# berkeley-hipie/HIPIE

Hardware: AMD Instinct MI355X
Metric: images/sec @1024x1024 ViT-H bs=8 (single-image inference hot path: box, class and mask logits) (higher is better)
Workload: dtype f16x3 (split-fp16 operands, fp32 accumulate: fp32-class); 1 GPU; BASELINE.json configs[2]: vit_huge, 1024x1024, batch 8 per GPU, 80 class prompts (L=194), detection; global_batch=8, parallelism=dp1, precision_policy=split, launch=eager

## Files before the change

### hipie_amd/_lib.py

```python
import ctypes
import os

_HERE = os.path.dirname(os.path.abspath(__file__))
LIB_PATH = os.environ.get("HIPIE_LIB_PATH") or os.path.join(_HERE, "csrc", "libhipie_mi355.so")

c_p = ctypes.c_void_p
c_i = ctypes.c_int
c_l = ctypes.c_int64
c_f = ctypes.c_float

SIGNATURES = {
    "hipie_version": [],
    "hipie_last_error": [],
    "hipie_msda_forward": [c_p, c_p, c_p, c_p, c_p, c_p] + [c_i] * 8 + [c_p],
    "hipie_msda_fused_forward": [c_p, c_p, c_p, c_p, c_p, c_p, c_p] + [c_i] * 10 + [c_l, c_l, c_p],
    "hipie_msda_fused_forward_strided": [c_p, c_l, c_p, c_p, c_p, c_p, c_p, c_p] + [c_i] * 10 + [c_l, c_l, c_p],
    "hipie_flash_attn": [c_p, c_p, c_p, c_p] + [c_i] * 5 + [c_l] * 12 + [c_p, c_p, c_i, c_i, c_p, c_f, c_f, c_i, c_p],
    "hipie_vit_attn": [c_p, c_p, c_p, c_p] + [c_i] * 5 + [c_f, c_i, c_p],
    "hipie_vit_attn_fused": [c_p, c_p, c_p, c_p] + [c_i] * 5 + [c_f, c_i, c_p],
    "hipie_vit_attn_rel": [c_p, c_p, c_p, c_p] + [c_i] * 7 + [c_p],
    "hipie_bi_xattn": [c_p, c_p, c_p, c_p, c_p, c_p, c_p] + [c_i] * 5 + [c_f, c_i, c_p],
    "hipie_bi_xattn_ws": [c_p, c_p, c_p, c_p, c_p, c_p, c_p, c_p, c_l] + [c_i] * 5 + [c_f, c_i, c_p],
    "hipie_bi_xattn_workspace": [c_i] * 5,
    "hipie_mask_einsum": [c_p, c_p, c_p] + [c_i] * 6 + [c_p],
    "hipie_mask_einsum_workspace": [c_i, c_i, c_i],
    "hipie_mask_einsum_ws": [c_p, c_p, c_p, c_p, c_p, c_l] + [c_i] * 6 + [c_p],
    "hipie_mask_einsum16": [c_p, c_p, c_p, c_p, c_p] + [c_i] * 6 + [c_p],
    "hipie_dynamic_mask": [c_p, c_p, c_p, c_p] + [c_i] * 7 + [c_p],
    "hipie_dynamic_mask16": [c_p, c_p, c_p, c_p] + [c_i] * 7 + [c_p],
    "hipie_dynamic_mask_backward": [c_p] * 7 + [c_i] * 6 + [c_p],
    "hipie_vit_relpos": [c_p, c_p, c_p, c_p, c_p] + [c_i] * 6 + [c_p],
    "hipie_add_layernorm": [c_p, c_p, c_p, c_p, c_p, c_p, c_l, c_i, c_f, c_i, c_i, c_i, c_p],
    "hipie_add_layernorm_sum": [c_p, c_p, c_p, c_p, c_p, c_p, c_p, c_p, c_l, c_i, c_f, c_i, c_i, c_i, c_p],
    "hipie_add_layernorm_rows": [c_p, c_p, c_p, c_p, c_p, c_p, c_l, c_i, c_f, c_i, c_i, c_i, c_p, c_p, c_p],
    "hipie_batched_nms": [c_p, c_p, c_p, c_p, c_p, c_i, c_i, c_f, c_i, c_p],
    "hipie_mask_finalize": [c_p, c_i, c_p] + [c_i] * 8 + [c_f, c_p, c_p],
    "hipie_sem_pan": [c_p] * 8 + [c_i] * 11 + [c_p],
    "hipie_sine_embed": [c_p, c_p, c_p, c_l, c_i, c_i, c_i, c_f, c_i, c_p],
    "hipie_box_refine": [c_p, c_p, c_p, c_l, c_f, c_i, c_p],
    "hipie_ref_point_mlp": [c_p, c_p, c_p, c_p, c_p, c_p, c_p, c_l, c_i, c_f, c_i, c_p],
    "hipie_box_head": [c_p, c_p, c_p, c_p, c_p, c_p, c_p, c_p, c_p, c_l, c_f, c_p],
    "hipie_add_layernorm_dec": [c_p, c_p, c_p, c_p, c_p, c_p, c_p, c_p, c_l, c_i, c_f, c_i, c_i, c_p],
    "hipie_add_cast": [c_p, c_p, c_p, c_l, c_i, c_p],
    "hipie_group_norm": [c_p, c_p, c_p, c_p, c_p, c_p, c_i, c_i, c_i, c_i, c_i, c_f, c_i, c_i, c_i, c_p],
    "hipie_gemm": [c_p, c_l, c_p, c_l, c_p, c_p, c_l, c_p, c_l, c_p] + [c_i] * 6 + [c_f, c_f, c_p],
    "hipie_gemm_f8x": [c_p, c_l, c_p, c_l, c_p, c_p, c_p, c_l, c_p, c_l, c_p] + [c_i] * 6 + [c_f, c_f, c_p],
    "hipie_to_f8x": [c_p, c_l, c_p, c_l, c_p, c_l, c_i, c_p],
    "hipie_gemm_ln": [c_p, c_l, c_p, c_l, c_p, c_p, c_l, c_p, c_p, c_f, c_p, c_l, c_p, c_l, c_i, c_i, c_i, c_f, c_p],
    "hipie_gemm_gather": [c_p, c_l, c_l, c_p, c_p, c_l, c_p, c_p, c_l, c_p, c_l, c_p] + [c_i] * 6 + [c_f, c_f, c_p],
    "hipie_vit_attn_split": [c_p, c_p, c_p, c_p] + [c_i] * 5 + [c_p],
    "hipie_msda_backward": [c_p] * 9 + [c_i] * 8 + [c_p],
    "hipie_msda_backward_ws": [c_p] * 9 + [c_i] * 8 + [c_p, c_l, c_p],
    "hipie_msda_backward_workspace": [c_i] * 6,
    "hipie_gemm_batched": [c_p, c_l, c_l, c_l, c_p, c_l, c_l, c_l, c_p, c_l, c_l, c_l] + [c_i] * 6 + [c_f, c_p],
    "hipie_gemm_batched_softmax_bias": [c_p, c_l, c_l, c_l, c_p, c_l, c_l, c_l, c_p, c_l, c_l, c_l] + [c_i] * 5 + [c_p, c_i, c_p, c_f, c_f, c_p],
    "hipie_gemm_batched_resid": [c_p, c_l, c_l, c_l, c_p, c_l, c_l, c_l, c_p, c_p, c_l, c_l, c_l, c_p, c_l, c_l, c_l] + [c_i] * 5 + [c_f, c_p],
    "hipie_gemm_batched_softmax": [c_p, c_l, c_l, c_l, c_p, c_l, c_l, c_l, c_p, c_l, c_l, c_l] + [c_i] * 5 + [c_p, c_i, c_f, c_f, c_p],
    "hipie_softmax_hl8": [c_p, c_l, c_p, c_l, c_l, c_i, c_i, c_p, c_l, c_f, c_p],
    "hipie_attn_f32": [c_p] * 5 + [c_i] * 5 + [c_l] * 6 + [c_f, c_p],
    "hipie_attn_split": [c_p] * 5 + [c_i] * 5 + [c_l] * 6 + [c_f, c_p],
    "hipie_attn_f32_rows": [c_p] * 5 + [c_i] * 5 + [c_l] * 6 + [c_f, c_p],
    "hipie_attn_split_rows": [c_p] * 5 + [c_i] * 5 + [c_l] * 6 + [c_f, c_p],
    "hipie_conv3x3_split": [c_p, c_l, c_p, c_p, c_p, c_l, c_l] + [c_i] * 6 + [c_p],
    "hipie_ffn_fused": [c_p, c_l, c_p, c_p, c_p, c_p, c_p, c_l, c_i, c_i, c_i, c_p],
    "hipie_topk": [c_p, c_l, c_i, c_i, c_i, c_p, c_p, c_p],
    "hipie_fill_rows": [c_p, c_l, c_p, c_l, c_p, c_l, c_p],
    "hipie_to_hl8": [c_p, c_l, c_p, c_l, c_l, c_i, c_i, c_f, c_p],
    "hipie_to_hl8_t": [c_p, c_l, c_p, c_l, c_l, c_i, c_l, c_f, c_p],
    "hipie_attn_train_forward": [c_p] * 8 + [c_i, c_i, c_p],
    "hipie_to_f16_pair": [c_p, c_l, c_p, c_p, c_l, c_i, c_i, c_p, c_p],
    "hipie_attn_train_backward": [c_p] * 13 + [c_i, c_i, c_p],
    "hipie_selftest": [c_i, c_p, c_p, c_p, c_p],
}

_lib = None


class HipieLibraryError(RuntimeError):
    pass


def load():
    global _lib
    if _lib is not None:
        return _lib
    if not os.path.exists(LIB_PATH):
        raise HipieLibraryError(
            "libhipie_mi355.so not found at %s -- build it with `make -C hipie_amd/csrc` (hipcc, gfx950). "
            "There is no PyTorch fallback for the hand-written kernels." % LIB_PATH)
    import torch
    try:
        lib = ctypes.CDLL(LIB_PATH)
    except OSError as e:
        raise HipieLibraryError("cannot load %s: %s" % (LIB_PATH, e))
    for name, argtypes in SIGNATURES.items():
        try:
            fn = getattr(lib, name)
        except AttributeError:
            raise HipieLibraryError("%s does not export %s (stale build?)" % (LIB_PATH, name))
        fn.argtypes = argtypes
        fn.restype = (ctypes.c_char_p if name == "hipie_last_error" else
                      ctypes.c_int64 if name in ("hipie_bi_xattn_workspace", "hipie_mask_einsum_workspace", "hipie_msda_backward_workspace") else ctypes.c_int)
    _lib = lib
    return lib


def check(rc, what):
    if rc != 0:
        msg = load().hipie_last_error()
        raise RuntimeError("%s failed (rc=%d): %s" % (what, rc, msg.decode() if msg else ""))
```

### hipie_amd/csrc/ffn_fused.hip

```cpp
#include "common.h"
#include "mfma.h"

namespace hipie {

struct FFParams {
  const char* X; const char* W1; const char* W2; const float* b1; const float* b2; float* out;
  long ldx_b, ldw1_b, ldw2_b, ldo;
  int M;
};

__device__ __forceinline__ void ff_dma16(const char* sbase, unsigned int voff, unsigned int lds_dst) {
#if defined(__HIP_DEVICE_COMPILE__)
  unsigned int keep;
  asm volatile("s_mov_b32 %0, m0\n\ts_mov_b32 m0, %3\n\ts_nop 0\n\tglobal_load_lds_dwordx4 %1, %2\n\ts_mov_b32 m0, %0"
               : "=&s"(keep) : "v"(voff), "s"(sbase), "s"(lds_dst) : "memory");
#endif
}

constexpr int FF_D = 256, FF_F = 2048, FF_C = 32;
constexpr int FF_W1B = FF_C * FF_D * 4;
constexpr int FF_W2B = FF_D * FF_C * 4;
constexpr int FF_BUF = FF_W1B + FF_W2B;

__global__ __launch_bounds__(256, 1) void ffn_fused_kernel(const FFParams p) {
  typedef f16_t T;
  typedef Mfma32<T>::frag frag;
  constexpr int KS = FF_D / 16;
  constexpr int NB = FF_D / 32;
  constexpr int NCH = FF_F / FF_C;
  extern __shared__ __attribute__((aligned(1024))) char smem[];
  float* sb1 = reinterpret_cast<float*>(smem + 2 * FF_BUF);

  const int tid = threadIdx.x, lane = tid & 63;
  const int wave = __builtin_amdgcn_readfirstlane(tid >> 6);
  const int li = lane & 31, hi = lane >> 5;
  const int m = blockIdx.x * 128 + wave * 32 + li;
  const int mc = min(m, p.M - 1);

  for (int i = tid; i < FF_F / 4; i += 256) reinterpret_cast<float4*>(sb1)[i] = reinterpret_cast<const float4*>(p.b1)[i];

  frag xh[KS], xl[KS];
  {
    const char* xr = p.X + (long)mc * p.ldx_b + 32 * hi;
#pragma unroll
    for (int ks = 0; ks < KS; ++ks) {
      xh[ks] = *reinterpret_cast<const frag*>(xr + 64 * ks);
      xl[ks] = *reinterpret_cast<const frag*>(xr + 64 * ks + 16);
    }
  }

  unsigned int dv1[8], dv2[8];
#pragma unroll
  for (int q = 0; q < 8; ++q) {
    const int i = wave + 4 * q;
    dv1[q] = (unsigned int)((long)i * p.ldw1_b + 16 * (lane ^ (i & 15)));
    const int f = 8 * i + (lane >> 3);
    dv2[q] = (unsigned int)((long)f * p.ldw2_b + 16 * ((lane & 7) ^ ((f >> 1) & 7)));
  }
  const unsigned int lds0 = (unsigned int)reinterpret_cast<uintptr_t>((__attribute__((address_space(3))) char*)smem);
  auto dma_chunk = [&](const int c, const int buf, const int q) {
    const int i = wave + 4 * q;
    ff_dma16(p.W1 + (long)c * FF_C * p.ldw1_b, dv1[q], __builtin_amdgcn_readfirstlane(lds0 + (unsigned int)(buf * FF_BUF + 1024 * i)));
    ff_dma16(p.W2 + (long)c * (FF_C * 4), dv2[q], __builtin_amdgcn_readfirstlane(lds0 + (unsigned int)(buf * FF_BUF + FF_W1B + 1024 * i)));
  };

  f32x16 acc[NB];
#pragma unroll
  for (int j = 0; j < NB; ++j)
#pragma unroll
    for (int r = 0; r < 16; ++r) acc[j][r] = 0.f;

#pragma unroll
  for (int q = 0; q < 8; ++q) dma_chunk(0, 0, q);

  const int w1row = li * 1024, w1sw = li & 15;
  const int w2row = FF_W1B + li * 128, w2sw = (li >> 1) & 7;

  for (int c = 0; c < NCH; ++c) {
    const int buf = c & 1;
    __builtin_amdgcn_s_waitcnt(0x0F70);
    __syncthreads();
    const char* bs = smem + buf * FF_BUF;
    const bool more = c + 1 < NCH;

    f32x16 h0, h1;
#pragma unroll
    for (int r = 0; r < 16; ++r) { h0[r] = 0.f; h1[r] = 0.f; }
#pragma unroll
    for (int ks = 0; ks < KS; ks += 2) {
      const frag ah0 = *reinterpret_cast<const frag*>(bs + w1row + 16 * ((2 * (2 * ks + hi)) ^ w1sw));
      const frag al0 = *reinterpret_cast<const frag*>(bs + w1row + 16 * ((2 * (2 * ks + hi) + 1) ^ w1sw));
      const frag ah1 = *reinterpret_cast<const frag*>(bs + w1row + 16 * ((2 * (2 * ks + 2 + hi)) ^ w1sw));
      const frag al1 = *reinterpret_cast<const frag*>(bs + w1row + 16 * ((2 * (2 * ks + 2 + hi) + 1) ^ w1sw));
      h0 = Mfma32<T>::mma(al0, xh[ks], h0);
      h1 = Mfma32<T>::mma(al1, xh[ks + 1], h1);
      h0 = Mfma32<T>::mma(ah0, xl[ks], h0);
      h1 = Mfma32<T>::mma(ah1, xl[ks + 1], h1);
      h0 = Mfma32<T>::mma(ah0, xh[ks], h0);
      h1 = Mfma32<T>::mma(ah1, xh[ks + 1], h1);
      if (more) dma_chunk(c + 1, buf ^ 1, ks >> 1);
    }
    frag Hh[2], Hl[2];
#pragma unroll
    for (int g = 0; g < 4; ++g) {
      const float4 b4 = *reinterpret_cast<const float4*>(sb1 + c * FF_C + 8 * g + 4 * hi);
      const float bb[4] = {b4.x, b4.y, b4.z, b4.w};
#pragma unroll
      for (int e = 0; e < 4; ++e) {
        const int r = 4 * g + e;
        T hh, ll;
        hl_split(fmaxf(h0[r] + h1[r] + bb[e], 0.f), hh, ll);
        Hh[r >> 3][r & 7] = hh;
        Hl[r >> 3][r & 7] = ll;
      }
    }
#pragma unroll
    for (int s2 = 0; s2 < 2; ++s2) {
      frag wh[NB], wl[NB];
#pragma unroll
      for (int j = 0; j < NB; ++j) {
        wh[j] = *reinterpret_cast<const frag*>(bs + w2row + j * 4096 + 16 * ((2 * (2 * s2 + hi)) ^ w2sw));
        wl[j] = *reinterpret_cast<const frag*>(bs + w2row + j * 4096 + 16 * ((2 * (2 * s2 + hi) + 1) ^ w2sw));
      }
#pragma unroll
      for (int j = 0; j < NB; ++j) acc[j] = Mfma32<T>::mma(wl[j], Hh[s2], acc[j]);
#pragma unroll
      for (int j = 0; j < NB; ++j) acc[j] = Mfma32<T>::mma(wh[j], Hl[s2], acc[j]);
#pragma unroll
      for (int j = 0; j < NB; ++j) acc[j] = Mfma32<T>::mma(wh[j], Hh[s2], acc[j]);
    }
  }

  if (m < p.M) {
    float* orow = p.out + (long)m * p.ldo;
#pragma unroll
    for (int j = 0; j < NB; ++j)
#pragma unroll
      for (int g = 0; g < 4; ++g) {
        const int n = 32 * j + 8 * g + 4 * hi;
        const float4 b4 = *reinterpret_cast<const float4*>(p.b2 + n);
        *reinterpret_cast<float4*>(orow + n) = make_float4(acc[j][4 * g] + b4.x, acc[j][4 * g + 1] + b4.y, acc[j][4 * g + 2] + b4.z, acc[j][4 * g + 3] + b4.w);
      }
  }
}

}

extern "C" int hipie_ffn_fused(const void* x, int64_t ldx, const void* w1, const float* b1, const void* w2p, const float* b2, float* out,
                               int64_t ldo, int M, int D, int F, void* stream) {
  using namespace hipie;
  HIPIE_REQUIRE(x && w1 && b1 && w2p && b2 && out, "ffn_fused: null pointer");
  HIPIE_REQUIRE(D == FF_D && F == FF_F, "ffn_fused: model width %d / hidden width %d (built for 256 / 2048)", D, F);
  HIPIE_REQUIRE(M > 0 && ldx >= 2 * D && ldx % 8 == 0 && ldo >= D && ldo % 4 == 0, "ffn_fused: M=%d ldx=%ld ldo=%ld", M, (long)ldx, (long)ldo);
  HIPIE_REQUIRE((((uintptr_t)x | (uintptr_t)w1 | (uintptr_t)w2p | (uintptr_t)b1 | (uintptr_t)b2 | (uintptr_t)out) & 15) == 0,
                "ffn_fused: pointers must be 16-byte aligned");
  FFParams p;
  p.X = (const char*)x; p.W1 = (const char*)w1; p.W2 = (const char*)w2p; p.b1 = b1; p.b2 = b2; p.out = out;
  p.ldx_b = ldx * 2; p.ldw1_b = (long)2 * D * 2; p.ldw2_b = (long)2 * F * 2; p.ldo = ldo;
  p.M = M;
  const size_t lds = (size_t)2 * FF_BUF + FF_F * sizeof(float);
  static bool lds_set[64] = {false};
  int dev = 0;
  (void)hipGetDevice(&dev);
  if (dev < 0 || dev >= 64 || !lds_set[dev]) {
    (void)hipFuncSetAttribute((const void*)ffn_fused_kernel, hipFuncAttributeMaxDynamicSharedMemorySize, (int)lds);
    if (dev >= 0 && dev < 64) lds_set[dev] = true;
  }
  hipLaunchKernelGGL(ffn_fused_kernel, dim3((unsigned)((M + 127) / 128)), dim3(256), lds, (hipStream_t)stream, p);
  return check_launch("ffn_fused");
}
```

### hipie_amd/ops.py

```python
import torch

from . import _lib

_DT = {torch.float32: 0, torch.float16: 1, torch.bfloat16: 2}
F32, F16, BF16, HL8 = 0, 1, 2, 4
OUT_F32 = 0x100
K_HL8_HI = 0x200


class _Profile(object):

    def __init__(self):
        self.tags, self.events = set(), {}
        self.shapes = False

    def enable(self, *tags):
        self.tags, self.events = set(tags), {}

    def disable(self):
        self.tags = set()

    def begin(self, tag):
        if tag not in self.tags and "all" not in self.tags:
            return None
# ... 1009 lines not shown
        lead = (M,)
        if out is not None and out_row is None and out.numel() // out.shape[-1] < M:
            raise RuntimeError("gemm: `out` has fewer rows (%d) than the row map (%d)" % (out.numel() // out.shape[-1], M))
        if resid is not None and resid.numel() // N < M:
            raise RuntimeError("gemm: `resid` has fewer rows (%d) than the row map (%d)" % (resid.numel() // N, M))
    if out_row is not None:
        if out is None:
            lead = (int(out_rows),)
        if out_row.dtype != torch.int32 or out_row.numel() != M or not out_row.is_contiguous():
            raise RuntimeError("gemm: out_row must be a contiguous int32 vector with one entry per row of a")
    if out is None:
        if out_fmt == F32:
            out = torch.empty(*lead, N, dtype=torch.float32, device=a.device)
        elif out_fmt == F16:
            out = torch.empty(*lead, N, dtype=torch.float16, device=a.device)
        else:
            out = torch.empty(*lead, 2 * N, dtype=torch.float16, device=a.device)
    o2 = out.reshape(-1, out.shape[-1])
    r2 = None
    if resid is not None:
        r2 = resid.reshape(-1, N)
        if r2.dtype != torch.float32 or r2.stride(-1) != 1:
            raise RuntimeError("gemm: resid must be fp32 with contiguous rows")
    if bias is not None and (bias.dtype != torch.float32 or not bias.is_contiguous()):
        raise RuntimeError("gemm: bias must be contiguous fp32")
    if a_row is not None:
        rc = lib.hipie_gemm_gather(a2.data_ptr(), a2.stride(0), a2.shape[0], a_row.data_ptr(), _chk(w, "w"), w.shape[1],
                                   None if bias is None else bias.data_ptr(), None if r2 is None else r2.data_ptr(), 0 if r2 is None else r2.stride(0),
                                   o2.data_ptr(), o2.stride(0), None if out_row is None else out_row.data_ptr(), M, N, Kw,
                                   F32 if a_f32 else HL8, int(out_fmt), int(act), float(alpha), float(oscale), _stream())
        _lib.check(rc, "hipie_gemm_gather")
        return out
    rc = lib.hipie_gemm(a2.data_ptr(), a2.stride(0), _chk(w, "w"), w.shape[1], None if bias is None else bias.data_ptr(),
                        None if r2 is None else r2.data_ptr(), 0 if r2 is None else r2.stride(0), o2.data_ptr(), o2.stride(0),
                        None if out_row is None else out_row.data_ptr(), M, N, Kw, F32 if a_f32 else (HL8 if split else F16), int(out_fmt), int(act), float(alpha), float(oscale), _stream())
    _lib.check(rc, "hipie_gemm")
    return out


@_timed(lambda qkv, tab_h, tab_w, grid_hw, heads: "vit_attn_global" if grid_hw[0] * grid_hw[1] > 256 else "vit_attn_window")
def vit_attn_split(qkv, tab_h, tab_w, grid_hw, heads):
    lib = _lib.load()
    gh, gw = grid_hw
    B, N, C6 = qkv.shape
    hd = C6 // (6 * heads)
    if qkv.dtype != torch.float16 or tab_h.dtype != torch.float16 or tab_w.dtype != torch.float16:
        raise RuntimeError("vit_attn_split: HL8 (fp16) operands expected")
    out = torch.empty(B, N, 2 * heads * hd, dtype=torch.float16, device=qkv.device)
    rc = lib.hipie_vit_attn_split(_chk(qkv, "qkv"), _chk(tab_h, "tab_h"), _chk(tab_w, "tab_w"), out.data_ptr(), B, gh, gw, heads, hd, _stream())
    _lib.check(rc, "hipie_vit_attn_split")
    return out


@_timed("gemm_split_k")
def gemm_split_k(a_hl8, w_hl8, nk):
    lib = _lib.load()
    M, K2 = a_hl8.shape
    N = w_hl8.shape[0]
    K = K2 // 2
    if w_hl8.shape[1] != K2 or K % (32 * nk) or a_hl8.dtype != torch.float16 or w_hl8.dtype != torch.float16 or not a_hl8.is_cuda:
        raise RuntimeError("gemm_split_k: HL8 device operands (M, 2K) / (N, 2K), K a multiple of 32 * nk")
    if N % 8:
        raise RuntimeError("gemm_split_k: N must be a multiple of 8")
    Kc = K // nk
    part = torch.empty(nk, M, N, dtype=torch.float32, device=a_hl8.device)
    rc = lib.hipie_gemm_batched(a_hl8.data_ptr(), K2, 0, 2 * Kc, w_hl8.data_ptr(), K2, 0, 2 * Kc, part.data_ptr(), N, 0, M * N, 1, nk, M, N, Kc,
                                F32, 1.0, _stream())
    _lib.check(rc, "hipie_gemm_batched")
    return part.sum(0)


@_timed("gemm_batched")
def matmul_nt_batched(a, w, alpha=1.0):
    lib = _lib.load()
    B, M, K = a.shape
    N = w.shape[1]
    if w.shape[0] != B or w.shape[2] != K or K % 32 or not a.is_cuda:
        raise RuntimeError("matmul_nt_batched: a (B, M, K), w (B, N, K) device tensors with K %% 32 == 0, got %s / %s" % (tuple(a.shape), tuple(w.shape)))
    Np = (N + 7) // 8 * 8
    if Np != N:
        wp = torch.zeros(B, Np, K, dtype=torch.float32, device=w.device)
        wp[:, :N] = w
        w = wp
    ah, wh = to_hl8(a.float().contiguous()), to_hl8(w.float().contiguous())
    out = torch.empty(B, M, Np, dtype=torch.float32, device=a.device)
    rc = lib.hipie_gemm_batched(ah.data_ptr(), 2 * K, M * 2 * K, 0, wh.data_ptr(), 2 * K, Np * 2 * K, 0, out.data_ptr(), Np, M * Np, 0,
                                B, 1, M, Np, K, F32, float(alpha), _stream())
    _lib.check(rc, "hipie_gemm_batched")
    return out if Np == N else out[..., :N]


def vit_attn_split_ok(grid_hw, hd):
    gh, gw = grid_hw

    def rows_ok(kh, kw):
        return (kw <= 32 and kh <= 160) or (kw <= 64 and kh <= 132) or (64 < kw <= 96 and kh <= 160)
    return hd in (64, 80) and ((gw == 14 and gh <= 96) or rows_ok(gh, gw) or (gw > 96 and gh <= 96 and rows_ok(gw, gh)))


def split_weight(owner, key, params, weight_fn, bias_fn=None):
    ver = tuple((q.data_ptr(), q._version, str(q.device)) for q in params)
    cache = owner.__dict__.setdefault("_hl8_cache", {})
    e = cache.get(key)
    if e is None or e[0] != ver:
        w = weight_fn().detach().float()
        b = None if bias_fn is None else bias_fn()
        b = None if b is None else b.detach().float()
        N = w.shape[0]
        Np = (N + 7) // 8 * 8
        if Np != N:
            w = torch.nn.functional.pad(w, (0, 0, 0, Np - N))
            b = None if b is None else torch.nn.functional.pad(b, (0, Np - N))
        e = (ver, hl8_pack(w), None if b is None else b.contiguous(), N)
        cache[key] = e
    return e[1], e[2], e[3]


def conv3x3_split_ok(x, conv):
    return (x.is_cuda and x.dim() == 4 and conv.kernel_size == (3, 3) and conv.stride == (1, 1) and conv.padding == (1, 1) and conv.dilation == (1, 1)
            and conv.padding_mode == "zeros" and conv.groups == 1 and conv.weight.dtype == torch.float32 and conv.in_channels % 32 == 0 and conv.out_channels % 256 == 0
            and x.shape[0] * (x.shape[2] + 2) * (x.shape[3] + 2) >= 16384)


_CONV_STAGE = {}
_RETIRED = []


@_timed("conv3x3_split")
def conv3x3_split(x, conv, act=ACT_NONE):
    lib = _lib.load()
    B, C, H, W = x.shape
    N = conv.out_channels
    Hp, Wp = H + 2, W + 2
    guard = Wp + 1
    rows = B * Hp * Wp
    skey = (B, C, H, W, str(x.device), torch.cuda.current_stream(x.device).cuda_stream)
    buf = _CONV_STAGE.get(skey)
    if buf is None:
        if len(_CONV_STAGE) >= 8:
            _RETIRED.append(_CONV_STAGE.pop(next(iter(_CONV_STAGE))))
        buf = _CONV_STAGE[skey] = torch.zeros(rows + 2 * guard, C, dtype=torch.float32, device=x.device)
    buf[guard:guard + rows].view(B, Hp, Wp, C)[:, 1:-1, 1:-1].copy_(x.permute(0, 2, 3, 1))
    w, b, _ = split_weight(conv, "w3x3", [conv.weight] + ([conv.bias] if conv.bias is not None else []),
                           lambda: conv.weight.permute(0, 2, 3, 1).reshape(N, 9 * C), (lambda: conv.bias) if conv.bias is not None else None)
    out = torch.empty(rows, N, dtype=torch.float32, device=x.device)
    xin = buf[guard:]
    rc = lib.hipie_conv3x3_split(xin.data_ptr(), C, w.data_ptr(), None if b is None else b.data_ptr(), out.data_ptr(), N, rows, Wp, C, N,
                                 F32, F32, int(act), _stream())
    _lib.check(rc, "hipie_conv3x3_split")
    return out.view(B, Hp, Wp, N)[:, 1:-1, 1:-1].permute(0, 3, 1, 2).contiguous(memory_format=torch.channels_last)


_FFN_PERM = {}


def ffn_fused_ok(x_hl8, lin1, lin2):
    return (x_hl8.is_cuda and lin1.weight.shape == (2048, 256) and lin2.weight.shape == (256, 2048) and lin1.bias is not None
            and lin2.bias is not None and lin1.weight.dtype == torch.float32 and x_hl8.numel() // 512 >= 4096)


@_timed("ffn_fused")
def ffn_fused(x_hl8, lin1, lin2):
    lib = _lib.load()
    w1, b1, _ = split_weight(lin1, "w", [lin1.weight, lin1.bias], lambda: lin1.weight, lambda: lin1.bias)
    F_ = lin2.weight.shape[1]
    perm = _FFN_PERM.get(F_)
    if perm is None:
        base = torch.tensor([0, 1, 2, 3, 8, 9, 10, 11, 4, 5, 6, 7, 12, 13, 14, 15])
        perm = _FFN_PERM[F_] = (torch.arange(0, F_, 16)[:, None] + base[None, :]).reshape(-1)
    w2, b2, _ = split_weight(lin2, "w_ffn_perm", [lin2.weight, lin2.bias], lambda: lin2.weight[:, perm.to(lin2.weight.device)], lambda: lin2.bias)
    lead = x_hl8.shape[:-1]
    x2 = x_hl8.reshape(-1, x_hl8.shape[-1])
    if x2.dtype != torch.float16 or x2.stride(-1) != 1 or x2.shape[-1] != 512:
        raise RuntimeError("ffn_fused: x must be HL8 rows of 2 * 256 fp16 values")
    M = x2.shape[0]
    out = torch.empty(M, 256, dtype=torch.float32, device=x2.device)
    rc = lib.hipie_ffn_fused(x2.data_ptr(), x2.stride(0), w1.data_ptr(), b1.data_ptr(), w2.data_ptr(), b2.data_ptr(), out.data_ptr(), 256,
                             M, 256, F_, _stream())
    _lib.check(rc, "hipie_ffn_fused")
    return out.view(*lead, 256)


def split_ok(K):
    return K % 32 == 0


def split_linear(x, owner, key, weight, bias=None, act=ACT_NONE, out_fmt=F32, resid=None, x_hl8=False, weight_fn=None, bias_fn=None,
                 tag="gemm", params=None, out=None, out_row=None, a_row=None):
    if params is None:
        params = [weight] + ([bias] if bias is not None else [])
    w, b, N = split_weight(owner, key, params, weight_fn or (lambda: weight), bias_fn or ((lambda: bias) if bias is not None else None))
    if x_hl8:
        a = x
    elif x.dtype == torch.float32 and x.stride(-1) == 1 and x.data_ptr() % 16 == 0 and (x.dim() < 2 or x.stride(-2) % 4 == 0):
        a = x if x.dim() <= 2 or x.is_contiguous() else x.contiguous()
    else:
        a = to_hl8(x if x.dtype in (torch.float32, torch.float16) else x.float())
    if out is not None or out_row is not None or a_row is not None:
        if N != w.shape[0]:
            raise RuntimeError("split_linear: in-place / row-mapped outputs need N % 8 == 0")
        return gemm(a, w, b, resid, out_fmt=out_fmt, act=act, split=True, tag=tag, out=out, out_row=out_row, a_row=a_row)
    out = gemm(a, w, b, resid, out_fmt=out_fmt, act=act, split=True, tag=tag)
    if N != w.shape[0]:
        out = out[..., :(2 * N if out_fmt == HL8 else N)].contiguous()
    return out



@_timed("to_f8x")
def to_f8x(x_hl8):
    lib = _lib.load()
    if x_hl8.dtype != torch.float16 or not x_hl8.is_cuda or x_hl8.shape[-1] % 64:
        raise RuntimeError("to_f8x: HL8 rows (fp16, 2K columns with K a multiple of 32) on the device")
    x2 = x_hl8.reshape(-1, x_hl8.shape[-1])
    if x2.stride(-1) != 1:
        x2 = x2.contiguous()
    R, K = x2.shape[0], x2.shape[1] // 2
    q = torch.empty(R, 2 * K, dtype=torch.uint8, device=x_hl8.device)
    sc = torch.empty(R, K // 32, 2, dtype=torch.uint8, device=x_hl8.device)
    rc = lib.hipie_to_f8x(x2.data_ptr(), x2.stride(0), q.data_ptr(), 2 * K, sc.data_ptr(), R, K, _stream())
    _lib.check(rc, "hipie_to_f8x")
    return q, sc


def f8x_weight(owner, key, params, weight_fn, bias_fn=None):
    from . import fp8x
    ver = tuple((q.data_ptr(), q._version, str(q.device)) for q in params)
    cache = owner.__dict__.setdefault("_f8x_cache", {})
    e = cache.get(key)
    if e is None or e[0] != ver:
        w = weight_fn().detach().float()
        b = None if bias_fn is None else bias_fn()
        b = None if b is None else b.detach().float()
        N = w.shape[0]
        Np = (N + 7) // 8 * 8
        if Np != N:
            w = torch.nn.functional.pad(w, (0, 0, 0, Np - N))
            b = None if b is None else torch.nn.functional.pad(b, (0, Np - N))
        w_hl8 = hl8_pack(w)
        q, sc = to_f8x(w_hl8) if w_hl8.is_cuda else (None, None)
        w8, wsc = fp8x.pack_from_hl8(w_hl8, q, sc)
        e = (ver, w8, wsc, None if b is None else b.contiguous(), N)
        cache[key] = e
    return e[1], e[2], e[3], e[4]


@_timed("gemm_f8x")
def gemm_f8x(a, w8, wsc, bias=None, resid=None, out_fmt=F32, act=ACT_NONE, alpha=1.0, oscale=1.0, out=None, out_row=None, out_rows=None):
    lib = _lib.load()
    if a.dtype != torch.float16 or w8.dtype != torch.uint8 or wsc.dtype != torch.uint8 or not a.is_cuda:
        raise RuntimeError("gemm_f8x: a HL8 (fp16) rows, w8 / wsc uint8, on the device")
    N, K = w8.shape[0], w8.shape[1] // 4
    a2 = a if a.dim() == 2 else a.reshape(-1, a.shape[-1])
    if a2.stride(-1) != 1 or a2.shape[-1] != 2 * K or not w8.is_contiguous() or tuple(wsc.shape) != (N, K // 32, 2) or not wsc.is_contiguous():
        raise RuntimeError("gemm_f8x: a rows %s against an f8x weight %s / scales %s" % (tuple(a.shape), tuple(w8.shape), tuple(wsc.shape)))
    M = a2.shape[0]
    lead = a.shape[:-1]
    if out_row is not None:
        if out is None:
            lead = (int(out_rows),)
        if out_row.dtype != torch.int32 or out_row.numel() != M or not out_row.is_contiguous():
            raise RuntimeError("gemm_f8x: out_row must be a contiguous int32 vector with one entry per row of a")
    if out is None:
        dt, width = {F32: (torch.float32, N), F16: (torch.float16, N), HL8: (torch.float16, 2 * N)}[out_fmt]
        out = torch.empty(*lead, width, dtype=dt, device=a.device)
    o2 = out.reshape(-1, out.shape[-1])
    r2 = None
    if resid is not None:
        r2 = resid.reshape(-1, N)
        if r2.dtype != torch.float32 or r2.stride(-1) != 1:
            raise RuntimeError("gemm_f8x: resid must be fp32 with contiguous rows")
    if bias is not None and (bias.dtype != torch.float32 or not bias.is_contiguous()):
        raise RuntimeError("gemm_f8x: bias must be contiguous fp32")
    rc = lib.hipie_gemm_f8x(a2.data_ptr(), a2.stride(0), _chk(w8, "w8"), 2 * K, _chk(wsc, "wsc"), None if bias is None else bias.data_ptr(),
                            None if r2 is None else r2.data_ptr(), 0 if r2 is None else r2.stride(0), o2.data_ptr(), o2.stride(0),
                            None if out_row is None else out_row.data_ptr(), M, N, K, HL8, int(out_fmt), int(act), float(alpha), float(oscale), _stream())
    _lib.check(rc, "hipie_gemm_f8x")
    return out


def f8x_linear(x_hl8, owner, key, weight, bias=None, act=ACT_NONE, out_fmt=F32, resid=None, out=None):
    params = [weight] + ([bias] if bias is not None else [])
    w8, wsc, b, N = f8x_weight(owner, key, params, lambda: weight, (lambda: bias) if bias is not None else None)
    if N != w8.shape[0]:
        raise RuntimeError("f8x_linear: N %% 8 == 0 expected (got %d)" % N)
    return gemm_f8x(x_hl8, w8, wsc, b, resid, out_fmt=out_fmt, act=act, out=out)

def split_linear_ln_ok(x, weight, norm_weight):
    return (x.is_cuda and weight.dtype == torch.float32 and weight.shape[0] == 256 and norm_weight.numel() == 256 and weight.shape[1] % 32 == 0
            and not torch.is_grad_enabled())


@_timed("gemm_ln")
def split_linear_ln(x, owner, key, weight, bias, resid, norm_weight, norm_bias, eps, x_hl8=False, want_hl8=True):
    lib = _lib.load()
    w, b, N = split_weight(owner, key, [weight] + ([bias] if bias is not None else []), lambda: weight, (lambda: bias) if bias is not None else None)
    if N != 256 or w.shape[0] != 256:
        raise RuntimeError("split_linear_ln: 256 output features expected")
    K = w.shape[1] // 2
    a_f32 = not x_hl8
    if a_f32 and (x.dtype != torch.float32 or x.stride(-1) != 1):
        raise RuntimeError("split_linear_ln: x must be fp32 rows or HL8")
    a2 = x.reshape(-1, x.shape[-1])
    if a2.shape[-1] != (K if a_f32 else 2 * K) or (a_f32 and (a2.stride(0) % 4 or a2.data_ptr() % 16)):
        raise RuntimeError("split_linear_ln: operand rows %s against weight %s" % (tuple(x.shape), tuple(weight.shape)))
    r2 = resid.reshape(-1, 256)
    M = a2.shape[0]
    if r2.dtype != torch.float32 or r2.stride(-1) != 1 or r2.shape[0] != M or not r2.is_cuda:
        raise RuntimeError("split_linear_ln: resid must be (rows, 256) fp32 on the device")
    out = torch.empty(*resid.shape[:-1], 256, dtype=torch.float32, device=x.device)
    o16 = torch.empty(*resid.shape[:-1], 512, dtype=torch.float16, device=x.device) if want_hl8 else None
    rc = lib.hipie_gemm_ln(a2.data_ptr(), a2.stride(0), _chk(w, "w"), w.shape[1], None if b is None else b.data_ptr(), r2.data_ptr(), r2.stride(0),
                           _chk(norm_weight, "norm_weight", torch.float32), _chk(norm_bias, "norm_bias", torch.float32), float(eps),
                           out.data_ptr(), 256, None if o16 is None else o16.data_ptr(), 512, M, K, F32 if a_f32 else HL8, 1.0, _stream())
    _lib.check(rc, "hipie_gemm_ln")
    return out, o16


_SHUFFLE_MAPS = {}


def _shuffle_maps(B, H, W, device):
    key = (B, H, W, str(device))
    m = _SHUFFLE_MAPS.get(key)
    if m is None:
        b = torch.arange(B, device=device).view(B, 1, 1)
        h = torch.arange(H, device=device).view(1, H, 1)
        w = torch.arange(W, device=device).view(1, 1, W)
        m = [((b * 2 * H + 2 * h + i) * 2 * W + 2 * w + j).reshape(-1).to(torch.int32).contiguous() for i in range(2) for j in range(2)]
        if len(_SHUFFLE_MAPS) > 16:
            _RETIRED.extend(_SHUFFLE_MAPS.values())
# ... 36 lines not shown
```

### include/hipie_mi355.h

```cpp
#ifndef HIPIE_MI355_H
#define HIPIE_MI355_H

#include <stdint.h>

#ifdef __cplusplus
extern "C" {
#endif

#define HIPIE_ABI_VERSION 13

#define HIPIE_F32 0
#define HIPIE_F16 1
#define HIPIE_BF16 2
#define HIPIE_F64 3
#define HIPIE_HL8 4

#define HIPIE_OUT_F32 0x100
#define HIPIE_K_HL8_HI 0x200

#define HIPIE_ATTN_FAST 1

#define HIPIE_OK 0
#define HIPIE_EINVAL (-22)
#define HIPIE_ELAUNCH (-5)
// ... 34 lines not shown

int hipie_vit_attn(const void* qkv, const float* rel_h, const float* rel_w, void* out,
                   int B, int gh, int gw, int heads, int hd, float scale, int dtype, void* stream);

int hipie_bi_xattn(const void* q, const void* k, const void* vv, const void* vl, const uint8_t* text_mask,
                   void* out_v, void* out_l, int B, int H, int Nv, int L, int hd, float clamp, int dtype, void* stream);

int64_t hipie_bi_xattn_workspace(int B, int H, int Nv, int L, int head_dim);
int hipie_bi_xattn_ws(const void* q, const void* k, const void* vv, const void* vl, const uint8_t* text_mask,
                      void* out_v, void* out_l, void* workspace, int64_t workspace_bytes, int B, int H, int Nv, int L,
                      int head_dim, float clamp, int dtype, void* stream);

int hipie_mask_einsum(const float* embed, const float* feats, void* out, int B, int Q, int C, int HW,
                      int precision, int out_dtype, void* stream);

int64_t hipie_mask_einsum_workspace(int B, int Q, int C);
int hipie_mask_einsum_ws(const float* embed, const float* feats, const float* row_bias, void* out, void* workspace,
                         int64_t workspace_bytes, int B, int Q, int C, int HW, int precision, int out_dtype, void* stream);

int hipie_mask_einsum16(const void* embed_hi, const void* embed_lo, const void* feats, const float* row_bias, void* out, int B,
                        int Q, int C, int HW, int dtype, int out_dtype, void* stream);

int hipie_dynamic_mask(const float* feats, const float* refs, const float* params, void* out,
                       int B, int Q, int H, int W, int stride, int up, int out_dtype, void* stream);

int hipie_dynamic_mask_backward(const float* feats, const float* refs, const float* params, const float* grad_out, float* grad_feats,
                                float* grad_refs, float* grad_params, int B, int Q, int H, int W, int stride, int up, void* stream);

int hipie_dynamic_mask16(const float* feats, const float* refs, const float* params, void* out,
                         int B, int Q, int H, int W, int stride, int dtype, int out_dtype, void* stream);

int hipie_vit_relpos(const void* qkv, const void* tab_h, const void* tab_w, float* rel_h, float* rel_w,
                     int B, int gh, int gw, int heads, int hd, int dtype, void* stream);

int hipie_add_layernorm(const void* x, const void* delta, const float* gamma, const float* beta, void* res_out,
                        void* norm_out, int64_t rows, int C, float eps, int x_dtype, int delta_dtype, int norm_dtype,
                        void* stream);

int hipie_vit_attn_fused(const void* qkv, const void* tab_h, const void* tab_w, void* out, int B, int gh, int gw, int heads,
                         int hd, float scale, int dtype, void* stream);

int hipie_vit_attn_rel(const void* qkv, const void* tab_h, const void* tab_w, void* out, int B, int gh, int gw, int heads,
                       int hd, int dtype, int flags, void* stream);

int hipie_add_layernorm_rows(const void* x, const void* delta, const float* gamma, const float* beta, void* res_out,
                             void* norm_out, int64_t out_rows, int C, float eps, int x_dtype, int delta_dtype,
                             int norm_dtype, const int32_t* delta_row, const int32_t* out_src, void* stream);

int hipie_add_layernorm_sum(const void* x, const void* delta, const float* gamma, const float* beta, void* res_out,
                            void* norm_out, const void* addend, void* sum_out, int64_t rows, int C, float eps,
                            int x_dtype, int delta_dtype, int norm_dtype, void* stream);

int hipie_add_layernorm_dec(const float* x, const void* delta, const float* gamma, const float* beta, float* norm_out,
                            void* norm16_out, const void* addend, void* sum16_out, int64_t rows, int C, float eps,
                            int delta_dtype, int aux_dtype, void* stream);

int hipie_ref_point_mlp(const float* ref, const float* dim_t, const void* w1t, const void* b1, const void* w2t, const void* b2,
                        void* out, int64_t n, int ref_stride, float scale, int dtype, void* stream);
int hipie_box_head(const float* x, const float* ref, const float* w1t, const float* b1, const float* w2t, const float* b2,
                   const float* w3t, const float* b3, float* out, int64_t n, float eps, void* stream);

int hipie_group_norm(const void* x, const float* prebias, const float* gamma, const float* beta, void* out, float* workspace,
                     int B, int C, int HW, int groups, int channels_last, float eps, int relu, int x_dtype, int out_dtype,
                     void* stream);

int hipie_add_cast(const float* a, const void* b, void* out, int64_t n, int dtype, void* stream);

int hipie_batched_nms(const float* boxes, const int64_t* classes, const int32_t* order, int32_t* keep, int32_t* count,
                      int B, int Q, float iou_threshold, int coordinate_trick, void* stream);

int hipie_mask_finalize(const void* masks, int dtype, const int32_t* qidx, int n, int hm, int wm, int up, int crop_h,
                        int crop_w, int out_h, int out_w, float threshold, uint8_t* out, void* stream);

int hipie_sem_pan(const float* masks, const void* cls_hi, const void* cls_lo, const float* pscore, float* sem,
                  int32_t* pan_idx, uint8_t* pan_own, int32_t* area, int N, int Npad, int C, int hm, int wm, int up,
                  int crop_h, int crop_w, int out_h, int out_w, int precision, void* stream);

int hipie_sine_embed(const float* ref, const float* dim_t, void* out, int64_t n, int n_coord, int num_pos_feats, int ref_stride,
                     float scale, int out_dtype, void* stream);

int hipie_box_refine(const void* delta, const float* ref, float* out, int64_t n, float eps, int delta_dtype, void* stream);

int hipie_gemm(const void* A, int64_t lda, const void* W, int64_t ldw, const float* bias, const float* resid, int64_t ldr,
               void* out, int64_t ldo, const int32_t* out_row, int M, int N, int K, int in_fmt, int out_fmt, int act, float alpha,
               float oscale, void* stream);

int hipie_gemm_f8x(const void* A, int64_t lda, const void* W, int64_t ldw, const void* w_scale, const float* bias, const float* resid,
                   int64_t ldr, void* out, int64_t ldo, const int32_t* out_row, int M, int N, int K, int in_fmt, int out_fmt, int act,
                   float alpha, float oscale, void* stream);

int hipie_to_f8x(const void* x, int64_t ldx, void* out, int64_t ldo, void* scale, int64_t rows, int K, void* stream);

int hipie_gemm_ln(const void* A, int64_t lda, const void* W, int64_t ldw, const float* bias, const float* resid, int64_t ldr,
                  const float* gamma, const float* beta, float eps, float* out, int64_t ldo, void* out_hl8, int64_t ldo_hl8, int M, int K,
                  int in_fmt, float alpha, void* stream);

int hipie_gemm_gather(const void* A, int64_t lda, int64_t a_rows, const int32_t* a_row, const void* W, int64_t ldw, const float* bias,
                      const float* resid, int64_t ldr, void* out, int64_t ldo, const int32_t* out_row, int M, int N, int K, int in_fmt,
                      int out_fmt, int act, float alpha, float oscale, void* stream);

int hipie_vit_attn_split(const void* qkv, const void* tab_h, const void* tab_w, void* out, int B, int gh, int gw, int heads,
                         int hd, void* stream);

int hipie_attn_train_forward(const void* q_hi, const void* q_lo, const void* k_hi, const void* k_lo, const void* v_hi, const void* v_lo,
                             void* out, void* lse, int BH, int N, void* stream);
int hipie_to_f16_pair(const void* x, int64_t ldx, void* hi, void* lo, int64_t rows, int C, int Cp, const void* scale, void* stream);
int hipie_attn_train_backward(const void* q_hi, const void* q_lo, const void* k_hi, const void* k_lo, const void* v_hi, const void* v_lo,
                              const void* do_hi, const void* do_lo, const void* lse, const void* delta, void* dq, void* dk, void* dv,
                              int BH, int N, void* stream);

int hipie_fill_rows(void* dst, int64_t ld_bytes, const int32_t* rows, int64_t n_rows, const void* src_row, int64_t row_bytes, void* stream);

int hipie_to_hl8(const void* x, int64_t ldx, void* out, int64_t ldo, int64_t rows, int K, int x_dtype, float scale, void* stream);

int hipie_to_hl8_t(const void* x, int64_t ldx, void* out, int64_t ldo, int64_t rows, int C, int64_t rows_p, float scale, void* stream);

int hipie_gemm_batched(const void* A, int64_t lda, int64_t a_outer, int64_t a_inner, const void* W, int64_t ldw, int64_t w_outer,
                       int64_t w_inner, void* out, int64_t ldo, int64_t o_outer, int64_t o_inner, int n_outer, int n_inner, int M, int N,
                       int K, int out_fmt, float alpha, void* stream);

int hipie_gemm_batched_softmax(const void* A, int64_t lda, int64_t a_outer, int64_t a_inner, const void* W, int64_t ldw, int64_t w_outer,
                               int64_t w_inner, void* out, int64_t ldo, int64_t o_outer, int64_t o_inner, int n_outer, int n_inner, int M,
                               int N, int K, const unsigned char* mask, int L, float clamp, float alpha, void* stream);

int hipie_gemm_batched_softmax_bias(const void* A, int64_t lda, int64_t a_outer, int64_t a_inner, const void* W, int64_t ldw, int64_t w_outer,
                                    int64_t w_inner, void* out, int64_t ldo, int64_t o_outer, int64_t o_inner, int n_outer, int n_inner,
                                    int M, int N, int K, const unsigned char* mask, int L, const float* col_bias, float clamp, float alpha,
                                    void* stream);
int hipie_gemm_batched_resid(const void* A, int64_t lda, int64_t a_outer, int64_t a_inner, const void* W, int64_t ldw, int64_t w_outer,
                             int64_t w_inner, const float* bias, const float* resid, int64_t ldr, int64_t r_outer, int64_t r_inner, float* out,
                             int64_t ldo, int64_t o_outer, int64_t o_inner, int n_outer, int n_inner, int M, int N, int K, float alpha,
                             void* stream);

int hipie_softmax_hl8(const float* S, int64_t lds, void* P, int64_t ldp, int64_t rows, int L, int Lp, const unsigned char* mask,
                      int64_t rows_per_batch, float clamp, void* stream);

int hipie_attn_f32(const float* q, const float* k, const float* v, const unsigned char* key_mask, float* out, int B, int H, int Nq, int Nk,
                   int head_dim, int64_t q_sb, int64_t q_st, int64_t k_sb, int64_t k_st, int64_t v_sb, int64_t v_st, float scale,
                   void* stream);

int hipie_attn_f32_rows(const float* q, const float* k, const float* v, const unsigned char* query_mask, float* out, int B, int H, int Nq,
                        int Nk, int head_dim, int64_t q_sb, int64_t q_st, int64_t k_sb, int64_t k_st, int64_t v_sb, int64_t v_st, float scale,
                        void* stream);
int hipie_attn_split_rows(const float* q, const float* k, const float* v, const unsigned char* query_mask, float* out, int B, int H, int Nq,
                          int Nk, int head_dim, int64_t q_sb, int64_t q_st, int64_t k_sb, int64_t k_st, int64_t v_sb, int64_t v_st, float scale,
                          void* stream);

int hipie_attn_split(const float* q, const float* k, const float* v, const unsigned char* key_mask, float* out, int B, int H, int Nq, int Nk,
                   int head_dim, int64_t q_sb, int64_t q_st, int64_t k_sb, int64_t k_st, int64_t v_sb, int64_t v_st, float scale,
                   void* stream);

int hipie_ffn_fused(const void* x, int64_t ldx, const void* w1, const float* b1, const void* w2p, const float* b2, float* out, int64_t ldo,
                    int M, int D, int F, void* stream);

int hipie_conv3x3_split(const void* x, int64_t ldx, const void* w, const float* bias, void* out, int64_t ldo, int64_t rows, int Wp, int C,
                        int N, int in_fmt, int out_fmt, int act, void* stream);

int hipie_topk(const float* x, int64_t row_stride, int rows, int n, int k, int64_t* idx_out, float* val_out, void* stream);

int hipie_selftest(int which, const uint16_t* a, const uint16_t* b, float* out, void* stream);

#ifdef __cplusplus
}
#endif
#endif
```

Baseline: 41.91 images/sec.

## Split tail tiles of fused FFN across hidden chunks with atomic reduction

```diff
diff --git a/hipie_amd/_lib.py b/hipie_amd/_lib.py
--- a/hipie_amd/_lib.py
+++ b/hipie_amd/_lib.py
@@ -63,6 +63,8 @@
     "hipie_attn_split_rows": [c_p] * 5 + [c_i] * 5 + [c_l] * 6 + [c_f, c_p],
     "hipie_conv3x3_split": [c_p, c_l, c_p, c_p, c_p, c_l, c_l] + [c_i] * 6 + [c_p],
     "hipie_ffn_fused": [c_p, c_l, c_p, c_p, c_p, c_p, c_p, c_l, c_i, c_i, c_i, c_p],
+    "hipie_ffn_fused_workspace": [c_i],
+    "hipie_ffn_fused_ws": [c_p, c_l, c_p, c_p, c_p, c_p, c_p, c_l, c_i, c_i, c_i, c_p, c_l, c_p],
     "hipie_topk": [c_p, c_l, c_i, c_i, c_i, c_p, c_p, c_p],
     "hipie_fill_rows": [c_p, c_l, c_p, c_l, c_p, c_l, c_p],
     "hipie_to_hl8": [c_p, c_l, c_p, c_l, c_l, c_i, c_i, c_f, c_p],
@@ -100,7 +102,8 @@
             raise HipieLibraryError("%s does not export %s (stale build?)" % (LIB_PATH, name))
         fn.argtypes = argtypes
         fn.restype = (ctypes.c_char_p if name == "hipie_last_error" else
-                      ctypes.c_int64 if name in ("hipie_bi_xattn_workspace", "hipie_mask_einsum_workspace", "hipie_msda_backward_workspace") else ctypes.c_int)
+                      ctypes.c_int64 if name in ("hipie_bi_xattn_workspace", "hipie_mask_einsum_workspace", "hipie_msda_backward_workspace",
+                                                  "hipie_ffn_fused_workspace") else ctypes.c_int)
     _lib = lib
     return lib
 
diff --git a/hipie_amd/csrc/ffn_fused.hip b/hipie_amd/csrc/ffn_fused.hip
--- a/hipie_amd/csrc/ffn_fused.hip
+++ b/hipie_amd/csrc/ffn_fused.hip
@@ -7,6 +7,8 @@
   const char* X; const char* W1; const char* W2; const float* b1; const float* b2; float* out;
   long ldx_b, ldw1_b, ldw2_b, ldo;
   int M;
+  int nfull, S;
+  float* part; unsigned int* cnt;
 };
 
 __device__ __forceinline__ void ff_dma16(const char* sbase, unsigned int voff, unsigned int lds_dst) {
@@ -34,7 +36,12 @@
   const int tid = threadIdx.x, lane = tid & 63;
   const int wave = __builtin_amdgcn_readfirstlane(tid >> 6);
   const int li = lane & 31, hi = lane >> 5;
-  const int m = blockIdx.x * 128 + wave * 32 + li;
+  const int bid = blockIdx.x;
+  const int tt = bid < p.nfull ? -1 : (bid - p.nfull) / p.S;
+  const int piece = bid < p.nfull ? 0 : (bid - p.nfull) - tt * p.S;
+  const int tile = bid < p.nfull ? bid : p.nfull + tt;
+  const int c0 = tt < 0 ? 0 : piece * NCH / p.S, c1 = tt < 0 ? NCH : (piece + 1) * NCH / p.S;
+  const int m = tile * 128 + wave * 32 + li;
   const int mc = min(m, p.M - 1);
 
   for (int i = tid; i < FF_F / 4; i += 256) reinterpret_cast<float4*>(sb1)[i] = reinterpret_cast<const float4*>(p.b1)[i];
@@ -71,17 +78,16 @@
     for (int r = 0; r < 16; ++r) acc[j][r] = 0.f;
 
 #pragma unroll
-  for (int q = 0; q < 8; ++q) dma_chunk(0, 0, q);
+  for (int q = 0; q < 8; ++q) dma_chunk(c0, 0, q);
 
   const int w1row = li * 1024, w1sw = li & 15;
   const int w2row = FF_W1B + li * 128, w2sw = (li >> 1) & 7;
 
-  for (int c = 0; c < NCH; ++c) {
-    const int buf = c & 1;
+  auto chunk = [&](const int c, const bool more) __attribute__((always_inline)) {
+    const int buf = (c - c0) & 1;
     __builtin_amdgcn_s_waitcnt(0x0F70);
     __syncthreads();
     const char* bs = smem + buf * FF_BUF;
-    const bool more = c + 1 < NCH;
 
     f32x16 h0, h1;
 #pragma unroll
@@ -129,6 +135,54 @@
 #pragma unroll
       for (int j = 0; j < NB; ++j) acc[j] = Mfma32<T>::mma(wh[j], Hh[s2], acc[j]);
     }
+  };
+  for (int c = c0; c < c1 - 1; ++c) chunk(c, true);
+  chunk(c1 - 1, false);
+
+  if (tt >= 0) {
+    auto partial = [&](const int s) { return reinterpret_cast<float4*>(p.part) + (long)(tt * p.S + s) * (NB * 4 * 256) + tid; };
+    float4* mine = partial(piece);
+#pragma unroll
+    for (int j = 0; j < NB; ++j)
+#pragma unroll
+      for (int g = 0; g < 4; ++g) mine[(4 * j + g) * 256] = make_float4(acc[j][4 * g], acc[j][4 * g + 1], acc[j][4 * g + 2], acc[j][4 * g + 3]);
+    asm volatile("s_waitcnt vmcnt(0)" ::: "memory");
+    __syncthreads();
+    int* flag = reinterpret_cast<int*>(sb1);
+    if (tid == 0) {
+      __builtin_amdgcn_fence(__ATOMIC_RELEASE, "agent");
+      asm volatile("s_waitcnt vmcnt(0)" ::: "memory");
+      const bool last = __hip_atomic_fetch_add(p.cnt + tt, 1u, __ATOMIC_RELAXED, __HIP_MEMORY_SCOPE_AGENT) == (unsigned int)(p.S - 1);
+      if (last) {
+        __builtin_amdgcn_fence(__ATOMIC_ACQUIRE, "agent");
+        asm volatile("s_waitcnt vmcnt(0)" ::: "memory");
+      }
+      *flag = last;
+    }
+    __syncthreads();
+    if (!*flag) return;
+    if (m >= p.M) return;
+    float4 t[NB * 4];
+#pragma unroll
+    for (int i = 0; i < NB * 4; ++i) t[i] = partial(0)[i * 256];
+    for (int s = 1; s < p.S; ++s) {
+      float4 f[NB * 4];
+#pragma unroll
+      for (int i = 0; i < NB * 4; ++i) f[i] = partial(s)[i * 256];
+#pragma unroll
+      for (int i = 0; i < NB * 4; ++i) { t[i].x += f[i].x; t[i].y += f[i].y; t[i].z += f[i].z; t[i].w += f[i].w; }
+    }
+    float* orow = p.out + (long)m * p.ldo;
+#pragma unroll
+    for (int j = 0; j < NB; ++j)
+#pragma unroll
+      for (int g = 0; g < 4; ++g) {
+        const int n = 32 * j + 8 * g + 4 * hi;
+        const float4 b4 = *reinterpret_cast<const float4*>(p.b2 + n);
+        const float4 v = t[4 * j + g];
+        *reinterpret_cast<float4*>(orow + n) = make_float4(v.x + b4.x, v.y + b4.y, v.z + b4.z, v.w + b4.w);
+      }
+    return;
   }
 
   if (m < p.M) {
@@ -146,9 +200,33 @@
 
 }
 
-extern "C" int hipie_ffn_fused(const void* x, int64_t ldx, const void* w1, const float* b1, const void* w2p, const float* b2, float* out,
-                               int64_t ldo, int M, int D, int F, void* stream) {
-  using namespace hipie;
+namespace {
+
+using namespace hipie;
+
+constexpr int FF_SMAX = 4;
+
+void ff_split(int M, int& nfull, int& S) {
+  static int ncu[64] = {0};
+  int dev = 0;
+  (void)hipGetDevice(&dev);
+  int n = dev >= 0 && dev < 64 ? ncu[dev] : 0;
+  if (n == 0) {
+    if (hipDeviceGetAttribute(&n, hipDeviceAttributeMultiprocessorCount, dev) != hipSuccess || n <= 0) n = 1;
+    if (dev >= 0 && dev < 64) ncu[dev] = n;
+  }
+  const int ntiles = (M + 127) / 128, r = ntiles % n;
+  S = r == 0 ? 1 : (n / r < FF_SMAX ? n / r : FF_SMAX);
+  if (S < 2) S = 1;
+  nfull = S == 1 ? ntiles : ntiles - r;
+}
+
+size_t ff_ws_bytes(int ntail, int S) {
+  return ntail == 0 ? 0 : (((size_t)ntail * sizeof(unsigned int) + 255) & ~(size_t)255) + (size_t)ntail * S * 128 * FF_D * sizeof(float);
+}
+
+int ff_launch(const void* x, int64_t ldx, const void* w1, const float* b1, const void* w2p, const float* b2, float* out, int64_t ldo,
+              int M, int D, int F, void* ws, int64_t ws_bytes, void* stream) {
   HIPIE_REQUIRE(x && w1 && b1 && w2p && b2 && out, "ffn_fused: null pointer");
   HIPIE_REQUIRE(D == FF_D && F == FF_F, "ffn_fused: model width %d / hidden width %d (built for 256 / 2048)", D, F);
   HIPIE_REQUIRE(M > 0 && ldx >= 2 * D && ldx % 8 == 0 && ldo >= D && ldo % 4 == 0, "ffn_fused: M=%d ldx=%ld ldo=%ld", M, (long)ldx, (long)ldo);
@@ -158,6 +236,23 @@
   p.X = (const char*)x; p.W1 = (const char*)w1; p.W2 = (const char*)w2p; p.b1 = b1; p.b2 = b2; p.out = out;
   p.ldx_b = ldx * 2; p.ldw1_b = (long)2 * D * 2; p.ldw2_b = (long)2 * F * 2; p.ldo = ldo;
   p.M = M;
+  const int ntiles = (M + 127) / 128;
+  p.nfull = ntiles; p.S = 1; p.part = nullptr; p.cnt = nullptr;
+  if (ws) {
+    int nfull, S;
+    ff_split(M, nfull, S);
+    const size_t need = ff_ws_bytes(ntiles - nfull, S);
+    HIPIE_REQUIRE(((uintptr_t)ws & 255) == 0, "ffn_fused: workspace must be 256-byte aligned");
+    HIPIE_REQUIRE((size_t)ws_bytes >= need, "ffn_fused: workspace of %ld bytes, %zu needed (hipie_ffn_fused_workspace)", (long)ws_bytes, need);
+    if (need > 0) {
+      p.nfull = nfull; p.S = S;
+      p.cnt = (unsigned int*)ws;
+      const size_t cbytes = need - (size_t)(ntiles - nfull) * S * 128 * FF_D * sizeof(float);
+      p.part = (float*)((char*)ws + cbytes);
+      if (hipMemsetAsync(ws, 0, (((size_t)(ntiles - nfull) * sizeof(unsigned int)) + 15) & ~(size_t)15, (hipStream_t)stream) != hipSuccess)
+        return set_err(HIPIE_ELAUNCH, "ffn_fused: hipMemsetAsync of the arrival counters failed");
+    }
+  }
   const size_t lds = (size_t)2 * FF_BUF + FF_F * sizeof(float);
   static bool lds_set[64] = {false};
   int dev = 0;
@@ -166,6 +261,28 @@
     (void)hipFuncSetAttribute((const void*)ffn_fused_kernel, hipFuncAttributeMaxDynamicSharedMemorySize, (int)lds);
     if (dev >= 0 && dev < 64) lds_set[dev] = true;
   }
-  hipLaunchKernelGGL(ffn_fused_kernel, dim3((unsigned)((M + 127) / 128)), dim3(256), lds, (hipStream_t)stream, p);
+  const int grid = p.nfull + (ntiles - p.nfull) * p.S;
+  hipLaunchKernelGGL(ffn_fused_kernel, dim3((unsigned)grid), dim3(256), lds, (hipStream_t)stream, p);
   return check_launch("ffn_fused");
 }
+
+}
+
+extern "C" int hipie_ffn_fused(const void* x, int64_t ldx, const void* w1, const float* b1, const void* w2p, const float* b2, float* out,
+                               int64_t ldo, int M, int D, int F, void* stream) {
+  return ff_launch(x, ldx, w1, b1, w2p, b2, out, ldo, M, D, F, nullptr, 0, stream);
+}
+
+extern "C" int64_t hipie_ffn_fused_workspace(int M) {
+  if (M <= 0) return 0;
+  int nfull, S;
+  ff_split(M, nfull, S);
+  return (int64_t)ff_ws_bytes((M + 127) / 128 - nfull, S);
+}
+
+extern "C" int hipie_ffn_fused_ws(const void* x, int64_t ldx, const void* w1, const float* b1, const void* w2p, const float* b2, float* out,
+                                  int64_t ldo, int M, int D, int F, void* workspace, int64_t workspace_bytes, void* stream) {
+  using namespace hipie;
+  HIPIE_REQUIRE(workspace, "ffn_fused_ws: null workspace (hipie_ffn_fused runs without one)");
+  return ff_launch(x, ldx, w1, b1, w2p, b2, out, ldo, M, D, F, workspace, workspace_bytes, stream);
+}
diff --git a/hipie_amd/ops.py b/hipie_amd/ops.py
--- a/hipie_amd/ops.py
+++ b/hipie_amd/ops.py
@@ -1185,6 +1185,11 @@
 
 
 _FFN_PERM = {}
+_FFN_WS = _Workspace()
+
+
+def ffn_tail_split_ok(M):
+    return True
 
 
 def ffn_fused_ok(x_hl8, lin1, lin2):
@@ -1208,8 +1213,14 @@
         raise RuntimeError("ffn_fused: x must be HL8 rows of 2 * 256 fp16 values")
     M = x2.shape[0]
     out = torch.empty(M, 256, dtype=torch.float32, device=x2.device)
-    rc = lib.hipie_ffn_fused(x2.data_ptr(), x2.stride(0), w1.data_ptr(), b1.data_ptr(), w2.data_ptr(), b2.data_ptr(), out.data_ptr(), 256,
-                             M, 256, F_, _stream())
+    need = int(lib.hipie_ffn_fused_workspace(M)) if ffn_tail_split_ok(M) else 0
+    if need > 0:
+        ws = _FFN_WS.get(need, x2.device)
+        rc = lib.hipie_ffn_fused_ws(x2.data_ptr(), x2.stride(0), w1.data_ptr(), b1.data_ptr(), w2.data_ptr(), b2.data_ptr(), out.data_ptr(),
+                                    256, M, 256, F_, ws.data_ptr(), ws.numel(), _stream())
+    else:
+        rc = lib.hipie_ffn_fused(x2.data_ptr(), x2.stride(0), w1.data_ptr(), b1.data_ptr(), w2.data_ptr(), b2.data_ptr(), out.data_ptr(), 256,
+                                 M, 256, F_, _stream())
     _lib.check(rc, "hipie_ffn_fused")
     return out.view(*lead, 256)
 
diff --git a/include/hipie_mi355.h b/include/hipie_mi355.h
--- a/include/hipie_mi355.h
+++ b/include/hipie_mi355.h
@@ -210,6 +210,9 @@
 
 int hipie_ffn_fused(const void* x, int64_t ldx, const void* w1, const float* b1, const void* w2p, const float* b2, float* out, int64_t ldo,
                     int M, int D, int F, void* stream);
+int64_t hipie_ffn_fused_workspace(int M);
+int hipie_ffn_fused_ws(const void* x, int64_t ldx, const void* w1, const float* b1, const void* w2p, const float* b2, float* out, int64_t ldo,
+                       int M, int D, int F, void* workspace, int64_t workspace_bytes, void* stream);
 
 int hipie_conv3x3_split(const void* x, int64_t ldx, const void* w, const float* bias, void* out, int64_t ldo, int64_t rows, int Wp, int C,
                         int N, int in_fmt, int out_fmt, int act, void* stream);
```

Result: no change. 41.57 images/sec (median of 2 runs) (-0.8%).
